# krg-nandu/monkey-pose

Hardware: NVIDIA B200
Metric: depth frames/sec (hGRU 8-step fwd) (higher is better)
Workload: dtype bf16

## Files before the change

monkey-pose_b200/csrc/hgru_lib.cu:

```cuda
#include "lib_common.cuh"

#include <cuda_bf16.h>
#include <cuda_fp16.h>
#include <cuda_runtime.h>

#include <atomic>
#include <cstdio>
#include <cstdlib>
#include <cstring>
#include <string>
#include <vector>

#include "crop.cuh"
#include "gate_tc.cuh"
#include "gemm_tc.cuh"
#include "post.cuh"
#include "hconv_tc.cuh"
#include "layers.cuh"
#include "simt_kernels.cuh"
#include <algorithm>

#include "attn.cuh"
#include "tc_host.cuh"

namespace {
thread_local std::string g_err;
int g_timing = 0;
}

namespace hgru_host {
int fail(int code, const std::string& msg) {
  g_err = msg;
  return code;
}
}

using namespace hgru_host;

namespace {

struct DevBuf {
  void* p = nullptr;
  size_t bytes = 0;
  int alloc(size_t b) {
    bytes = b;
    cudaError_t e = cudaMalloc(&p, b ? b : 16);
    if (e != cudaSuccess) return fail(HGRU_E_CUDA, std::string("cudaMalloc: ") + cudaGetErrorString(e));
    return 0;
  }
  void release() {
    if (p) cudaFree(p);
    p = nullptr;
  }
  template <class T> T* as() const { return static_cast<T*>(p); }
};

template <int KP, class Epi>
int launch_gate(const __nv_bfloat16* act, const hgru::TcConvArgs& a, cudaStream_t st) {
  using Cfg = hgru::GateCfg<KP>;
  const int tiles_per_frame = (a.H * a.W + 127) / 128;
  hgru::gate_tc_kernel<KP, Epi><<<a.N * tiles_per_frame, 128, Cfg::SMEM_BYTES, st>>>(act, a);
  CUDA_TRY(cudaGetLastError());
  return 0;
}
template <class Epi>
int dispatch_gate(int KP, const __nv_bfloat16* act, const hgru::TcConvArgs& a, cudaStream_t st) {
  if (KP == 64) return launch_gate<64, Epi>(act, a, st);
  if (KP == 32) return launch_gate<32, Epi>(act, a, st);
  if (KP == 16) return launch_gate<16, Epi>(act, a, st);
  return fail(HGRU_E_UNSUPPORTED, "tensor-core gate: unsupported padded channel count");
}

template <int S>
int launch_simt_conv(const float* in, const float* w, const float* bias, const float* scale,
                     const float* shift, float* out, int N, int H, int W, int Ci, int Co, int relu,
                     cudaStream_t st) {
  using Cfg = hgru::ConvSimtCfg<S>;
  auto kern = hgru::conv_simt_kernel<S>;
  SMEM_ATTR_ONCE(kern, Cfg::kSmemBytes);
  dim3 grid(((W + 15) / 16) * ((H + 15) / 16), (Co + 63) / 64, N);
  kern<<<grid, 256, Cfg::kSmemBytes, st>>>(in, w, bias, scale, shift, out, N, H, W, Ci, Co, relu);
  CUDA_TRY(cudaGetLastError());
  return 0;
}

int dispatch_simt_conv(int S, const float* in, const float* w, const float* bias, const float* scale,
                       const float* shift, float* out, int N, int H, int W, int Ci, int Co, int relu,
                       cudaStream_t st) {
  switch (S) {
    case 1: return launch_simt_conv<1>(in, w, bias, scale, shift, out, N, H, W, Ci, Co, relu, st);
    case 3: return launch_simt_conv<3>(in, w, bias, scale, shift, out, N, H, W, Ci, Co, relu, st);
    case 5: return launch_simt_conv<5>(in, w, bias, scale, shift, out, N, H, W, Ci, Co, relu, st);
    case 7: return launch_simt_conv<7>(in, w, bias, scale, shift, out, N, H, W, Ci, Co, relu, st);
    case 9: return launch_simt_conv<9>(in, w, bias, scale, shift, out, N, H, W, Ci, Co, relu, st);
    case 11: return launch_simt_conv<11>(in, w, bias, scale, shift, out, N, H, W, Ci, Co, relu, st);
    case 13: return launch_simt_conv<13>(in, w, bias, scale, shift, out, N, H, W, Ci, Co, relu, st);
    case 15: return launch_simt_conv<15>(in, w, bias, scale, shift, out, N, H, W, Ci, Co, relu, st);
    default: return fail(HGRU_E_UNSUPPORTED, "conv: filter size must be odd and <= 15");
  }
}

__global__ void pad_matrix_kernel(const float* in, float* out, int rows, int k, int KP, int rows_pad) {
  const int i = blockIdx.x * blockDim.x + threadIdx.x;
  if (i >= rows_pad * KP) return;
  const int c = i % KP, r = i / KP;
  out[i] = (r < rows && c < k) ? in[static_cast<size_t>(r) * k + c] : 0.f;
}
__global__ void pad_hwio_kernel(const float* in, float* out, int taps, int k, int KP) {
  const size_t i = blockIdx.x * static_cast<size_t>(blockDim.x) + threadIdx.x;
  if (i >= static_cast<size_t>(taps) * KP * KP) return;
  const int co = i % KP;
  const int ci = (i / KP) % KP;
  const int t = i / (static_cast<size_t>(KP) * KP);
  out[i] = (ci < k && co < k) ? in[(static_cast<size_t>(t) * k + ci) * k + co] : 0.f;
}

struct KernelTimer {
  std::vector<cudaEvent_t> ev;
  int used = 0;
  int kernels = 0;
  bool open = false;
  void begin(cudaStream_t st) {
    if (!g_timing || open) return;
    open = true;
    while (static_cast<int>(ev.size()) < used + 2) {
      cudaEvent_t e;
      cudaEventCreate(&e);
      ev.push_back(e);
    }
    cudaEventRecord(ev[used], st);
  }
  void end(cudaStream_t st, int n = 1) {
    if (!g_timing || !open) return;
    cudaEventRecord(ev[used + 1], st);
    used += 2;
    kernels += n;
    open = false;
  }
  void reset() { used = 0; kernels = 0; open = false; }
  int collect(float* total_ms) {
    float t = 0.f;
    for (int i = 0; i + 1 < used; i += 2) {
      cudaEventSynchronize(ev[i + 1]);
      float ms = 0.f;
      cudaEventElapsedTime(&ms, ev[i], ev[i + 1]);
      t += ms;
    }
    *total_ms = t;
    return used ? kernels : 0;
  }
  ~KernelTimer() {
    for (auto e : ev) cudaEventDestroy(e);
  }
// ... 629 lines not shown
    if (int r = p->h0_tmp.alloc(static_cast<size_t>(N) * HW * HW * C * sizeof(float))) return r;
  }
  if (h->op16() && !p->h0_identity) {
    if (!p->side_st) {
      CUDA_TRY(cudaStreamCreateWithFlags(&p->side_st, cudaStreamNonBlocking));
      CUDA_TRY(cudaEventCreateWithFlags(&p->ev_fork, cudaEventDisableTiming));
      CUDA_TRY(cudaEventCreateWithFlags(&p->ev_init, cudaEventDisableTiming));
    }
    CUDA_TRY(cudaEventRecord(p->ev_fork, st));
    CUDA_TRY(cudaStreamWaitEvent(p->side_st, p->ev_fork, 0));
    if ((rc = hgru_init_state_bf16(h, H2_init, p->side_st))) return rc;
    CUDA_TRY(cudaEventRecord(p->ev_init, p->side_st));
    h->state_ready = true;
  }
  const int per = (N + nchunks - 1) / nchunks;
  const size_t pix = static_cast<size_t>(HW) * HW;
  auto conv1 = [&](int n0, int nn) {
    float* o32 = tc ? nullptr : p->pool1.as<float>() + static_cast<size_t>(n0) * pix * KP;
    __nv_bfloat16* o16 = tc ? p->act_pool1.as<__nv_bfloat16>() + static_cast<size_t>(n0) * 2 * KP * pix : nullptr;
    hgru::stem_conv1_pool_bn_kernel<<<dim3(nblk(static_cast<size_t>(nn) * HW * ((HW + hgru::kStemPix - 1) / hgru::kStemPix)), KP / 8),
                                      256, 0, st>>>(
        depth + static_cast<size_t>(n0) * 4 * pix, p->w1.as<float>(), p->b1.as<float>(), p->bn_scale(0), p->bn_shift(0),
        o32, o16, nn, HW, HW, C, KP, tc ? 1 : 0);
    ++p->launches;
  };
  auto conv23_tc = [&](int n0, int nn) -> int {
    hgru::TcConvArgs a{};
    a.N = nn; a.n0 = n0; a.H = HW; a.W = HW; a.KP = KP; a.kreal = C;
    a.wpk = p->wpk2.as<__nv_bfloat16>(); a.bias = p->b2.as<float>();
    a.scale = p->bn_scale(1); a.shift = p->bn_shift(1);
    a.out = nullptr; a.out_bf16 = p->act_conv2.as<__nv_bfloat16>();
    int r = tc_stem_launch(KP, p->map_pool1, a, st);
    if (r) return r;
    a.wpk = p->wpk3.as<__nv_bfloat16>(); a.bias = p->b3.as<float>();
    a.scale = p->bn_scale(2); a.shift = p->bn_shift(2);
    a.out = h->Xp.as<float>(); a.out_bf16 = nullptr;
    p->launches += 2;
    return tc_stem_launch(KP, p->map_conv2, a, st);
  };
  for (int c = 0; c < nchunks; ++c) {
    const int n0 = c * per, nn = (n0 + per <= N ? per : N - n0);
    if (nn <= 0) break;
    if (chunk_ready) CUDA_TRY(cudaStreamWaitEvent(st, chunk_ready[c], 0));
    conv1(n0, nn);
    if (tc && (rc = conv23_tc(n0, nn))) return rc;
  }
  if (!tc) {
    if ((rc = dispatch_simt_conv(3, p->pool1.as<float>(), p->w2.as<float>(), p->b2.as<float>(), p->bn_scale(1),
                                 p->bn_shift(1), p->conv2.as<float>(), N, HW, HW, KP, KP, 1, st)))
      return rc;
    if ((rc = dispatch_simt_conv(3, p->conv2.as<float>(), p->w3.as<float>(), p->b3.as<float>(), p->bn_scale(2),
                                 p->bn_shift(2), h->Xp.as<float>(), N, HW, HW, KP, KP, 1, st)))
      return rc;
    p->launches += 2;
  }
  if (p->fc1_tc) {
    h->fc_a = p->fc1_a.as<__nv_bfloat16>(); h->fc_scale = p->bn_scale(3); h->fc_shift = p->bn_shift(3);
    h->fc_kpad = p->fc_kpad;
  }
  if (p->h0_identity) {
    state_to_nhwc(h, h->Xp.as<float>(), p->h0_tmp.as<float>(), st);
    H2_init = p->h0_tmp.as<float>();
    ++p->launches;
  } else if (h->op16()) {
    CUDA_TRY(cudaStreamWaitEvent(st, p->ev_init, 0));
  }
  if ((rc = hgru_run_padded(h, h->Xp.as<float>(), H2_init, nullptr, nullptr, st))) return rc;
  p->launches += h->launches;
  const int K = HW * HW * C;
  int nsplit = p->nsplit;
  if (p->fc1_tc) {
    hgru::GemmArgs g{N, p->F, K, p->fc_kpad, p->fc_kbps, p->part.as<float>(), 0, 0, 0, 0, 0, 0};
    dim3 grid((p->F + hgru::kGemmBN - 1) / hgru::kGemmBN, (N + hgru::kGemmBM - 1) / hgru::kGemmBM, p->fc_splits);
    hgru::gemm_tc_splitk_kernel<hgru::kGemmBN><<<grid, 256, hgru::kGemmSmemBytes, st>>>(p->map_fc_a, p->map_fc_a, p->map_fc_b, g);
    nsplit = p->fc_splits;
    ++p->launches;
  } else {
    const int kslice = round_up((K + p->nsplit - 1) / p->nsplit, 16);
    dim3 g1((p->F + 63) / 64, (N + 63) / 64, p->nsplit);
    hgru::fc1_splitk_kernel<<<g1, 256, 0, st>>>(h->H2.as<float>(), p->fc1_w.as<float>(), p->bn_scale(3),
                                                p->bn_shift(3), p->part.as<float>(), N, K, p->F, C, KP, kslice);
    ++p->launches;
  }
  hgru::fc_tail_kernel<<<N, 256, sizeof(float) * (p->F + hgru::kFcTailScratch), st>>>(
      p->part.as<float>(), nsplit, p->fc1_b.as<float>(), p->bn_scale(4), p->bn_shift(4),
      p->fc2_w.as<float>(), p->fc2_b.as<float>(), p->fc1.as<float>(), out, N, p->F, p->O);
  ++p->launches;
  CUDA_TRY(cudaGetLastError());
  return 0;
}

#include "attn_plan.inl"

extern "C" {

const char* hgru_last_error(void) { return g_err.c_str(); }
int hgru_version(void) { return 100; }
int hgru_enable_kernel_timing(int on) {
  g_timing = on ? 1 : 0;
  return 0;
}

int hgru_plan_create(int N, int H, int W, int k, int S, int T, int mode, hgru_plan_t* out) {
  if (!out) return fail(HGRU_E_INVALID, "hgru_plan_create: out is null");
  *out = nullptr;
  hgru_plan_s* p = new hgru_plan_s();
  int rc = hgru_plan_init(p, N, H, W, k, S, T, mode);
  if (!rc && cudaDeviceSynchronize() != cudaSuccess)
    rc = fail(HGRU_E_CUDA, "hgru_plan_create: device synchronisation failed");
  if (rc) {
    hgru_plan_free(p);
    delete p;
    return rc;
  }
  *out = p;
  return 0;
}

int hgru_plan_destroy(hgru_plan_t plan) {
  if (!plan) return 0;
  hgru_plan_free(plan);
  delete plan;
  return 0;
}

int hgru_set_params(hgru_plan_t plan, const float* p_r, const float* i_r, const float* i_b,
                    const float* o_r, const float* o_b, const float* beta, const float* nu,
                    const float* gamma, const float* kappa, const float* omega, const float* rho,
                    const float* lateral_bias, void* stream) {
  if (!plan) return fail(HGRU_E_INVALID, "hgru_set_params: null plan");
  return hgru_set_params_impl(plan, p_r, i_r, i_b, o_r, o_b, beta, nu, gamma, kappa, omega, rho,
                              lateral_bias, static_cast<cudaStream_t>(stream));
}

int hgru_forward(hgru_plan_t p, const float* X, const float* H2_init, float* H2_out, float* H1_trace,
                 float* H2_trace, void* stream) {
  if (!p) return fail(HGRU_E_INVALID, "hgru_forward: null plan");
  if (!X || !H2_out) return fail(HGRU_E_INVALID, "hgru_forward: null tensor pointer");
  cudaStream_t st = static_cast<cudaStream_t>(stream);
  state_from_nhwc(p, X, p->Xp.as<float>(), st);
  int rc = hgru_run_padded(p, p->Xp.as<float>(), H2_init, H1_trace, H2_trace, st);
  if (rc) return rc;
  state_to_nhwc(p, p->H2.as<float>(), H2_out, st);
  p->launches += 3;
  CUDA_TRY(cudaGetLastError());
  return 0;
}

size_t hgru_plan_workspace_bytes(hgru_plan_t plan) { return plan ? plan->workspace() : 0; }
int hgru_plan_launch_count(hgru_plan_t plan) { return plan ? plan->launches : 0; }

int pose_plan_create(int N, int HW, int C, int S, int T, int F, int O, int mode, pose_plan_t* out) {
  if (!out) return fail(HGRU_E_INVALID, "pose_plan_create: out is null");
  *out = nullptr;
  if (N < 1 || HW < 1 || C < 1 || F < 1 || O < 1) return fail(HGRU_E_INVALID, "pose_plan_create: non-positive shape");
  pose_plan_s* p = new pose_plan_s();
  p->N = N; p->HW = HW; p->C = C; p->S = S; p->T = T; p->F = F; p->O = O; p->mode = mode;
  int rc = hgru_plan_init(&p->hg, N, HW, HW, C, S, T, mode);
  const int KP = p->hg.KP;
  p->KP = KP;
  p->bnw = F > KP ? F : KP;
  const size_t act = static_cast<size_t>(N) * HW * HW * KP * sizeof(float);
  const size_t K = static_cast<size_t>(HW) * HW * C;
  auto A = [&](DevBuf& b, size_t bytes) { if (!rc) rc = b.alloc(bytes); };
  A(p->depth, static_cast<size_t>(N) * 4 * HW * HW * sizeof(float));
  if (mode == HGRU_MODE_FP32) { A(p->pool1, act); A(p->conv2, act); }
  A(p->w1, sizeof(float) * 9 * C); A(p->b1, sizeof(float) * KP);
  A(p->b2, sizeof(float) * KP); A(p->b3, sizeof(float) * KP);
  p->fc1_tc = (mode != HGRU_MODE_FP32);
// ... 526 lines not shown
```

monkey-pose_b200/csrc/simt_kernels.cuh:

```cuda
#pragma once
#include <cuda_bf16.h>
#include <cuda_fp16.h>
#include <cuda_runtime.h>

#include <cstdint>

#include "op_format.cuh"

namespace hgru {

__device__ __forceinline__ float sigmoidf_(float x) { return 1.f / (1.f + __expf(-x)); }
__device__ __forceinline__ float tanhf_(float x) { return tanhf(x); }

template <int S>
struct ConvSimtCfg {
  static constexpr int PH = 16 + S - 1;
  static constexpr int PWraw = 16 + S - 1;
  static constexpr int PW = ((8 + ((8 + S - 1 + 3) / 4) * 4) + 3) / 4 * 4;
  static constexpr int NWIN = ((8 + S - 1 + 3) / 4) * 4;
  static constexpr int kPatchFloats = 8 * PH * PW;
  static constexpr int kWFloats = S * 8 * 64;
  static constexpr int kSmemBytes = (kPatchFloats + kWFloats) * 4;
};

template <int S>
__global__ void __launch_bounds__(256)
conv_simt_kernel(const float* __restrict__ in, const float* __restrict__ w,
                 const float* __restrict__ bias, const float* __restrict__ scale,
                 const float* __restrict__ shift, float* __restrict__ out, int N, int H, int W,
                 int Ci, int Co, int relu) {
  using Cfg = ConvSimtCfg<S>;
  extern __shared__ float smem_f[];
  float* patch = smem_f;
  float* wsm = smem_f + Cfg::kPatchFloats;
  constexpr int PAD = (S - 1) / 2;
  const int tiles_x = (W + 15) / 16;
  const int tx = blockIdx.x % tiles_x, ty = blockIdx.x / tiles_x;
  const int co0 = blockIdx.y * 64;
  const int n = blockIdx.z;
  const int tid = threadIdx.x;
  const int cg = tid & 7;
  const int pg = tid >> 3;
  const int prow = pg >> 1;
  const int pxg = (pg & 1) * 8;
  const int y_base = ty * 16 - PAD, x_base = tx * 16 - PAD;

  float acc[8][8];
#pragma unroll
  for (int j = 0; j < 8; ++j)
#pragma unroll
    for (int c = 0; c < 8; ++c) acc[j][c] = 0.f;

  for (int ci0 = 0; ci0 < Ci; ci0 += 8) {
    __syncthreads();
    for (int e = tid; e < Cfg::PH * Cfg::PWraw * 8; e += 256) {
      const int ci = e & 7;
      const int p = e >> 3;
      const int px = p % Cfg::PWraw, py = p / Cfg::PWraw;
      const int y = y_base + py, x = x_base + px;
      float v = 0.f;
      if (y >= 0 && y < H && x >= 0 && x < W && ci0 + ci < Ci)
        v = in[((static_cast<size_t>(n) * H + y) * W + x) * Ci + ci0 + ci];
      patch[(ci * Cfg::PH + py) * Cfg::PW + px] = v;
    }
    for (int dy = 0; dy < S; ++dy) {
      __syncthreads();
      for (int e = tid; e < S * 8 * 64; e += 256) {
        const int co = e & 63;
        const int ci = (e >> 6) & 7;
        const int dx = e >> 9;
        float v = 0.f;
        if (ci0 + ci < Ci && co0 + co < Co)
          v = w[((static_cast<size_t>(dy) * S + dx) * Ci + ci0 + ci) * Co + co0 + co];
        wsm[e] = v;
      }
      __syncthreads();
#pragma unroll 1
      for (int ci = 0; ci < 8; ++ci) {
        float win[Cfg::NWIN];
        const float4* src =
            reinterpret_cast<const float4*>(patch + (ci * Cfg::PH + prow + dy) * Cfg::PW + pxg);
#pragma unroll
        for (int j = 0; j < Cfg::NWIN / 4; ++j) {
          const float4 v = src[j];
          win[4 * j] = v.x; win[4 * j + 1] = v.y; win[4 * j + 2] = v.z; win[4 * j + 3] = v.w;
        }
#pragma unroll
        for (int dx = 0; dx < S; ++dx) {
          const float4* wp = reinterpret_cast<const float4*>(wsm + (dx * 8 + ci) * 64 + cg * 8);
          const float4 w0 = wp[0], w1 = wp[1];
// ... 472 lines not shown
        const int c = cg * 8 + j;
        g.v[j] = (c < k) ? sigmoidf_(acc[i][j] + bg[c]) : 0.f;
        const float a = g.v[j] * xin[pp * (KP + 1) + c];
        hi.v[j] = __bfloat162float(__float2bfloat16(a));
        lo.v[j] = a - hi.v[j];
      }
      if (out_g) {
        float* o = out_g + ((n * (KP >> 2) + 2 * cg) * HW + pin) * 4;
        *reinterpret_cast<float4*>(o) = make_float4(g.v[0], g.v[1], g.v[2], g.v[3]);
        *reinterpret_cast<float4*>(o + static_cast<size_t>(HW) * 4) = make_float4(g.v[4], g.v[5], g.v[6], g.v[7]);
      }
      if (out_act && lo_off) {
        st8_stacked(out_act, static_cast<int>(n), cg, CG, pin, HW, W, act_pad, hi);
        st8_stacked(out_act + lo_off, static_cast<int>(n), cg, CG, pin, HW, W, act_pad, lo);
      } else if (out_act) {
        st8_bf16(chunk_ptr(out_act, static_cast<int>(n), cg, pin, HW, 2 * CG), hi);
        st8_bf16(chunk_ptr(out_act, static_cast<int>(n), CG + cg, pin, HW, 2 * CG), lo);
      }
    }
  }
}

__global__ void __launch_bounds__(256)
fc1_splitk_kernel(const float* __restrict__ A, const float* __restrict__ Wt,
                  const float* __restrict__ sc, const float* __restrict__ sh,
                  float* __restrict__ part, int M, int K, int Nout, int kch, int KP, int kslice) {
  __shared__ float As[16][64 + 4];
  __shared__ float Bs[16][64 + 4];
  const int tid = threadIdx.x;
  const int j0 = blockIdx.x * 64, m0 = blockIdx.y * 64, z = blockIdx.z;
  const int kb = z * kslice, ke = min(K, kb + kslice);
  const int tm = (tid >> 4) * 4, tj = (tid & 15) * 4;
  float acc[4][4] = {};
  for (int k0 = kb; k0 < ke; k0 += 16) {
    {
      const int r = tid >> 2, kk = (tid & 3) * 4;
      const int m = m0 + r;
#pragma unroll
      for (int q = 0; q < 4; ++q) {
        const int kidx = k0 + kk + q;
        float v = 0.f;
        if (m < M && kidx < ke) {
          const int pix = kidx / kch, c = kidx - pix * kch;
          v = A[(static_cast<size_t>(m) * (K / kch) + pix) * KP + c] * sc[c] + sh[c];
        }
        As[kk + q][r] = v;
      }
    }
    {
      const int kk = tid >> 4, jj = (tid & 15) * 4;
      const int kidx = k0 + kk;
#pragma unroll
      for (int q = 0; q < 4; ++q) {
        const int j = j0 + jj + q;
        Bs[kk][jj + q] = (kidx < ke && j < Nout) ? Wt[static_cast<size_t>(kidx) * Nout + j] : 0.f;
      }
    }
    __syncthreads();
#pragma unroll
    for (int kk = 0; kk < 16; ++kk) {
      float a[4], b[4];
#pragma unroll
      for (int q = 0; q < 4; ++q) { a[q] = As[kk][tm + q]; b[q] = Bs[kk][tj + q]; }
#pragma unroll
      for (int q = 0; q < 4; ++q)
#pragma unroll
        for (int r = 0; r < 4; ++r) acc[q][r] = fmaf(a[q], b[r], acc[q][r]);
    }
    __syncthreads();
  }
#pragma unroll
  for (int q = 0; q < 4; ++q) {
    const int m = m0 + tm + q;
    if (m >= M) continue;
#pragma unroll
    for (int r = 0; r < 4; ++r) {
      const int j = j0 + tj + r;
      if (j < Nout) part[(static_cast<size_t>(z) * M + m) * Nout + j] = acc[q][r];
    }
  }
}

constexpr int kFcTailScratch = 256;
__global__ void __launch_bounds__(256)
fc_tail_kernel(const float* __restrict__ part, int nsplit, const float* __restrict__ b1,
               const float* __restrict__ sc, const float* __restrict__ sh,
               const float* __restrict__ W2, const float* __restrict__ b2, float* __restrict__ fc1_out,
               float* __restrict__ out, int M, int Hid, int Nout) {
  extern __shared__ float r[];
  float* scratch = r + Hid;
  const int m = blockIdx.x;
  const size_t zs = static_cast<size_t>(M) * Hid;
  if ((Hid & 3) == 0) {
    for (int j = 4 * threadIdx.x; j < Hid; j += 4 * blockDim.x) {
      const float* pj = part + static_cast<size_t>(m) * Hid + j;
      float4 a = make_float4(0.f, 0.f, 0.f, 0.f);
      int z = 0;
      for (; z + 6 <= nsplit; z += 6) {
        float4 v[6];
#pragma unroll
        for (int q = 0; q < 6; ++q) v[q] = __ldg(reinterpret_cast<const float4*>(pj + (z + q) * zs));
#pragma unroll
        for (int q = 0; q < 6; ++q) { a.x += v[q].x; a.y += v[q].y; a.z += v[q].z; a.w += v[q].w; }
      }
      for (; z < nsplit; ++z) {
        const float4 v = __ldg(reinterpret_cast<const float4*>(pj + z * zs));
        a.x += v.x; a.y += v.y; a.z += v.z; a.w += v.w;
      }
      const float av[4] = {a.x, a.y, a.z, a.w};
#pragma unroll
      for (int q = 0; q < 4; ++q) {
        const float t = av[q] + b1[j + q];
        if (fc1_out) fc1_out[static_cast<size_t>(m) * Hid + j + q] = t;
        r[j + q] = fmaxf(t, 0.f) * sc[j + q] + sh[j + q];
      }
    }
  } else {
    for (int j = threadIdx.x; j < Hid; j += blockDim.x) {
      const float* pj = part + static_cast<size_t>(m) * Hid + j;
      float a = 0.f;
      for (int z = 0; z < nsplit; ++z) a += pj[z * zs];
      a += b1[j];
      if (fc1_out) fc1_out[static_cast<size_t>(m) * Hid + j] = a;
      r[j] = fmaxf(a, 0.f) * sc[j] + sh[j];
    }
  }
  __syncthreads();
  for (int o0 = 0; o0 < Nout; o0 += kFcTailScratch) {
    const int no = min(Nout - o0, kFcTailScratch);
    const int G = kFcTailScratch / no;
    const int g = threadIdx.x / no, o = threadIdx.x - g * no;
    if (g < G) {
      const float* wcol = W2 + o0 + o;
      float acc[4] = {0.f, 0.f, 0.f, 0.f};
      int j = g;
      for (; j + 15 * G < Hid; j += 16 * G) {
        float w[16];
#pragma unroll
        for (int q = 0; q < 16; ++q) w[q] = __ldg(wcol + static_cast<size_t>(j + q * G) * Nout);
#pragma unroll
        for (int q = 0; q < 16; ++q) acc[q & 3] = fmaf(r[j + q * G], w[q], acc[q & 3]);
      }
      for (; j < Hid; j += G) acc[0] = fmaf(r[j], __ldg(wcol + static_cast<size_t>(j) * Nout), acc[0]);
      scratch[g * no + o] = (acc[0] + acc[1]) + (acc[2] + acc[3]);
    }
    __syncthreads();
    if (threadIdx.x < no) {
      float a = 0.f;
      for (int gg = 0; gg < G; ++gg) a += scratch[gg * no + threadIdx.x];
      out[static_cast<size_t>(m) * Nout + o0 + threadIdx.x] = a + b2[o0 + threadIdx.x];
    }
    __syncthreads();
  }
}

__global__ void bn_fold_kernel(const float* gamma, const float* beta, const float* mean,
                               const float* var, float eps, float* scale, float* shift, int c) {
  const int i = blockIdx.x * blockDim.x + threadIdx.x;
  if (i >= c) return;
  const float s = gamma[i] / sqrtf(var[i] + eps);
  scale[i] = s;
  shift[i] = beta[i] - mean[i] * s;
}

template <class F = OpBf16>
__global__ void pack_weights_kernel(const float* __restrict__ w, typename F::T* __restrict__ wpk,
                                    int taps, int k, int ksteps, int co_pad, int ci_wrap = 0) {
  const size_t i = blockIdx.x * static_cast<size_t>(blockDim.x) + threadIdx.x;
  const size_t total = static_cast<size_t>(ksteps) * taps * 2 * co_pad * 8;
  if (i >= total) return;
  const int j = i & 7;
  size_t r = i >> 3;
  const int co = r % co_pad; r /= co_pad;
  const int ch = r & 1; r >>= 1;
  const int tap = r % taps;
  const int q = r / taps;
  int ci = q * 16 + ch * 8 + j;
  if (ci_wrap > 0 && ci >= ci_wrap) ci -= ci_wrap;
  float v = 0.f;
  if (ci < k && co < k) v = w[(static_cast<size_t>(tap) * k + ci) * k + co];
  wpk[i] = F::cvt(v);
}

template <class F = OpBf16>
__global__ void pack_weights_pairtap_kernel(const float* __restrict__ w, typename F::T* __restrict__ wpk, int k,
                                            int ksteps) {
  const size_t i = blockIdx.x * static_cast<size_t>(blockDim.x) + threadIdx.x;
  const size_t total = static_cast<size_t>(ksteps) * 15 * 8 * 2 * 128 * 8;
  if (i >= total) return;
  const int j = i & 7;
  size_t r = i >> 3;
  const int row = r % 128; r /= 128;
  const int ch = r & 1; r >>= 1;
  const int b = r % 8; r /= 8;
  const int dy = r % 15;
  const int q = static_cast<int>(r / 15);
  int dx = -1;
  if (b == 0) { if (row < 64) dx = 7; }
  else dx = (row < 64) ? (b - 1 + 8) : (b - 1);
  const int co = row & 63;
  const int ci = q * 16 + ch * 8 + j;
  float v = 0.f;
  if (dx >= 0 && ci < k && co < k) v = w[((static_cast<size_t>(dy) * 15 + dx) * k + ci) * k + co];
  wpk[i] = F::cvt(v);
}

__global__ void pack_weights_split3_kernel(const float* __restrict__ w, __nv_bfloat16* __restrict__ wpk,
                                           int taps, int k, int ksteps, int co_pad) {
  const size_t i = blockIdx.x * static_cast<size_t>(blockDim.x) + threadIdx.x;
  const size_t group = static_cast<size_t>(3) * taps * 2 * co_pad * 8;
  if (i >= group * ksteps) return;
  const int q = static_cast<int>(i / group);
  size_t r = i - q * group;
  const size_t wide_elems = static_cast<size_t>(taps) * 2 * (2 * co_pad) * 8;
  int tap, ch, n, j, lo;
  if (r < wide_elems) {
    j = r & 7; r >>= 3;
    n = r % (2 * co_pad); r /= (2 * co_pad);
    ch = r & 1; tap = static_cast<int>(r >> 1);
    lo = n >= co_pad;
    if (lo) n -= co_pad;
  } else {
    r -= wide_elems;
    j = r & 7; r >>= 3;
    n = r % co_pad; r /= co_pad;
    ch = r & 1; tap = static_cast<int>(r >> 1);
    lo = 0;
  }
  const int ci = q * 16 + ch * 8 + j;
  float v = 0.f;
  if (ci < k && n < k) v = w[(static_cast<size_t>(tap) * k + ci) * k + n];
  const __nv_bfloat16 hi = __float2bfloat16(v);
  wpk[i] = lo ? __float2bfloat16(v - __bfloat162float(hi)) : hi;
// ... 4 lines not shown
```

monkey-pose_b200/csrc/sm100_ptx.cuh:

```cuda
#pragma once
#include <cstdint>
#include <cuda.h>

namespace sm100 {

__device__ __forceinline__ uint32_t smem_u32(const void* p) {
  return static_cast<uint32_t>(__cvta_generic_to_shared(p));
}

__device__ __forceinline__ bool elect_one() {
  uint32_t pred;
  asm volatile(
      "{\n\t.reg .pred p;\n\t"
      "elect.sync _|p, 0xffffffff;\n\t"
      "selp.u32 %0, 1, 0, p;\n\t}"
      : "=r"(pred));
  return pred != 0;
}

__device__ __forceinline__ void mbar_init(uint32_t bar, uint32_t count) {
  asm volatile("mbarrier.init.shared::cta.b64 [%0], %1;" ::"r"(bar), "r"(count) : "memory");
}
__device__ __forceinline__ void fence_barrier_init() {
  asm volatile("fence.mbarrier_init.release.cluster;" ::: "memory");
}
__device__ __forceinline__ void fence_proxy_async() {
  asm volatile("fence.proxy.async.shared::cta;" ::: "memory");
}
__device__ __forceinline__ void grid_launch_dependents() { asm volatile("griddepcontrol.launch_dependents;" ::: "memory"); }
__device__ __forceinline__ int ld_acquire_gpu(const int* p) {
  int v;
  asm volatile("ld.acquire.gpu.global.s32 %0, [%1];" : "=r"(v) : "l"(p) : "memory");
  return v;
}
__device__ __forceinline__ void fence_proxy_async_global() { asm volatile("fence.proxy.async.global;" ::: "memory"); }
__device__ __forceinline__ void mbar_arrive(uint32_t bar) {
  asm volatile("mbarrier.arrive.shared::cta.b64 _, [%0];" ::"r"(bar) : "memory");
}
__device__ __forceinline__ void mbar_arrive_expect_tx(uint32_t bar, uint32_t bytes) {
  asm volatile("mbarrier.arrive.expect_tx.shared::cta.b64 _, [%0], %1;" ::"r"(bar), "r"(bytes)
               : "memory");
}
__device__ __forceinline__ bool mbar_try_wait(uint32_t bar, uint32_t parity) {
  uint32_t ok;
  asm volatile(
      "{\n\t.reg .pred p;\n\t"
      "mbarrier.try_wait.parity.shared::cta.b64 p, [%1], %2;\n\t"
      "selp.u32 %0, 1, 0, p;\n\t}"
      : "=r"(ok)
      : "r"(bar), "r"(parity)
      : "memory");
  return ok != 0;
}
__device__ __forceinline__ bool mbar_test(uint32_t bar, uint32_t parity) {
  uint32_t ok;
  asm volatile(
      "{\n\t.reg .pred p;\n\t"
      "mbarrier.test_wait.parity.shared::cta.b64 p, [%1], %2;\n\t"
      "selp.u32 %0, 1, 0, p;\n\t}"
      : "=r"(ok)
      : "r"(bar), "r"(parity)
      : "memory");
  return ok != 0;
}
__device__ __forceinline__ void mbar_wait(uint32_t bar, uint32_t parity) {
  while (!mbar_try_wait(bar, parity)) {
  }
}
__device__ __forceinline__ void mbar_wait_warp(uint32_t bar, uint32_t parity) {
  while (!__all_sync(0xffffffffu, mbar_try_wait(bar, parity))) {
  }
}

__device__ __forceinline__ void tma_prefetch_desc(const CUtensorMap* m) {
  asm volatile("prefetch.tensormap [%0];" ::"l"(reinterpret_cast<uint64_t>(m)) : "memory");
}
__device__ __forceinline__ void tma_load_4d(uint32_t dst, const CUtensorMap* m, uint32_t bar,
                                            int c0, int c1, int c2, int c3) {
  asm volatile(
      "cp.async.bulk.tensor.4d.shared::cluster.global.mbarrier::complete_tx::bytes"
      " [%0], [%1, {%3, %4, %5, %6}], [%2];"
      ::"r"(dst), "l"(reinterpret_cast<uint64_t>(m)), "r"(bar), "r"(c0), "r"(c1), "r"(c2), "r"(c3)
      : "memory");
}
__device__ __forceinline__ void tma_load_2d(uint32_t dst, const CUtensorMap* m, uint32_t bar,
                                            int c0, int c1) {
  asm volatile(
      "cp.async.bulk.tensor.2d.shared::cluster.global.mbarrier::complete_tx::bytes"
      " [%0], [%1, {%3, %4}], [%2];"
      ::"r"(dst), "l"(reinterpret_cast<uint64_t>(m)), "r"(bar), "r"(c0), "r"(c1)
      : "memory");
}
__device__ __forceinline__ void bulk_load(uint32_t dst, const void* src, uint32_t bytes,
                                          uint32_t bar) {
  asm volatile(
      "cp.async.bulk.shared::cluster.global.mbarrier::complete_tx::bytes [%0], [%1], %2, [%3];"
      ::"r"(dst), "l"(reinterpret_cast<uint64_t>(src)), "r"(bytes), "r"(bar)
      : "memory");
}

template <uint32_t kCols>
__device__ __forceinline__ void tmem_alloc(uint32_t slot_smem) {
  asm volatile("tcgen05.alloc.cta_group::1.sync.aligned.shared::cta.b32 [%0], %1;"
               ::"r"(slot_smem), "n"(kCols) : "memory");
  asm volatile("tcgen05.relinquish_alloc_permit.cta_group::1.sync.aligned;" ::: "memory");
}
template <uint32_t kCols>
__device__ __forceinline__ void tmem_dealloc(uint32_t taddr) {
  asm volatile("tcgen05.dealloc.cta_group::1.sync.aligned.b32 %0, %1;" ::"r"(taddr), "n"(kCols)
               : "memory");
}
__device__ __forceinline__ void tc_fence_before() {
// ... 121 lines not shown
```

Measured before the change: 51950.

## Batch multiple frames per fc tail block and chain it with programmatic launch

The readout tail kernel now handles up to four frames per block with 512 threads. Two thread halves each cover interleaved frames, so every loaded FC2 weight is reused across several frames instead of being re-read per frame. The kernel is launched with programmatic stream serialization after the tensor-core split-K GEMM and waits on griddepcontrol, which lets its launch overlap the GEMM tail. Unroll depths for the split-sum and weight loops are also increased. The cost is more shared memory and registers per block and fewer blocks in the grid. A profiling script is also added.

```diff
diff --git a/monkey-pose_b200/csrc/devtools/step_breakdown.py b/monkey-pose_b200/csrc/devtools/step_breakdown.py
--- /dev/null
+++ b/monkey-pose_b200/csrc/devtools/step_breakdown.py
@@ -0,0 +1,148 @@
+import argparse
+import json
+import os
+import subprocess
+import sys
+import tempfile
+
+sys.path.insert(0, os.path.join(os.path.dirname(os.path.abspath(__file__)), "..", "..", ".."))
+import torch
+from torch.profiler import ProfilerActivity, profile
+
+import monkey_pose_b200 as mp
+from monkey_pose_b200 import initialization as init
+
+
+def gpu_info():
+    q = "name,power.limit,clocks.max.sm"
+    try:
+        row = subprocess.run(["nvidia-smi", "-i", str(torch.cuda.current_device()), "--query-gpu=" + q,
+                              "--format=csv,noheader"], capture_output=True, text=True, timeout=30).stdout.strip()
+        name, power, clk = [x.strip() for x in row.split(",")]
+        return {"gpu": name, "power_limit": power, "sm_clock_max": clk}
+    except Exception as e:
+        return {"gpu": torch.cuda.get_device_name(), "power_limit": "unknown (%r)" % e, "sm_clock_max": None}
+
+
+def phase_of(name, seen_hgru):
+    if "init_state" in name:
+        return "init"
+    if "stem_conv1" in name:
+        return "conv1"
+    if "hconv_stack_kernel" in name:
+        return "hgru"
+    if "hconv_tc_kernel" in name:
+        return "hgru" if seen_hgru else "conv23"
+    if "gemm_tc_splitk" in name:
+        return "fc1"
+    if "fc_tail" in name:
+        return "tail"
+    return "other"
+
+
+def median(xs):
+    xs = sorted(xs)
+    return xs[len(xs) // 2] if xs else None
+
+
+def main():
+    ap = argparse.ArgumentParser()
+    ap.add_argument("--batch", type=int, default=256)
+    ap.add_argument("--channels", type=int, default=25)
+    ap.add_argument("--timesteps", type=int, default=8)
+    ap.add_argument("--mode", default="bf16")
+    ap.add_argument("--steps", type=int, default=20)
+    ap.add_argument("--warmup", type=int, default=5)
+    ap.add_argument("--out", help="also write the result as JSON to this file")
+    a = ap.parse_args()
+    assert torch.cuda.is_available(), "step_breakdown.py measures on a CUDA device"
+
+    P = init.pose_params(channels=a.channels, S=15, T=a.timesteps, hw=64, fc_hidden=1024, out=69, seed=3)
+    depth = torch.as_tensor(init.synthetic_depth(a.batch, seed=1234)).cuda()
+    m = mp.model()
+    m.channels, m.timesteps, m.compute_mode = a.channels, a.timesteps, a.mode
+    m.hidden_state = torch.as_tensor(init.hidden_init((a.batch, 64, 64, a.channels), seed=5)).cuda()
+    m.load_params(P)
+    for _ in range(a.warmup):
+        m.build(depth, 69)
+    torch.cuda.synchronize()
+
+    e0, e1 = torch.cuda.Event(enable_timing=True), torch.cuda.Event(enable_timing=True)
+    e0.record()
+    for _ in range(a.steps):
+        m.build(depth, 69)
+    e1.record()
+    torch.cuda.synchronize()
+    step_ms = e0.elapsed_time(e1) / a.steps
+
+    with profile(activities=[ProfilerActivity.CUDA]) as prof:
+        for _ in range(a.steps):
+            torch.cuda._sleep(100)
+            m.build(depth, 69)
+        torch.cuda._sleep(100)
+        torch.cuda.synchronize()
+    with tempfile.TemporaryDirectory() as d:
+        trace = os.path.join(d, "trace.json")
+        prof.export_chrome_trace(trace)
+        with open(trace) as f:
+            events = json.load(f)["traceEvents"]
+    kern = sorted((e for e in events if e.get("cat") == "kernel"), key=lambda e: e["ts"])
+    steps, cur = [], None
+    for e in kern:
+        if "spin_kernel" in e["name"]:
+            if cur:
+                steps.append(cur)
+            cur = []
+        elif cur is not None:
+            cur.append(e)
+    per_step = []
+    for ks in steps:
+        seen_hgru, rows = False, []
+        for e in ks:
+            ph = phase_of(e["name"], seen_hgru)
+            seen_hgru |= ph == "hgru"
+            rows.append((ph, float(e["ts"]), float(e["ts"]) + float(e["dur"])))
+        if not any(r[0] == "hgru" for r in rows):
+            continue
+        t_first = min(r[1] for r in rows)
+        busy = {}
+        for ph, s, t in rows:
+            b = busy.setdefault(ph, [0.0, 0])
+            b[0] += t - s
+            b[1] += 1
+        hg = [r for r in rows if r[0] == "hgru"]
+        h0, h1 = min(r[1] for r in hg), max(r[2] for r in hg)
+        fc_end = max((r[2] for r in rows if r[0] == "fc1"), default=h1)
+        end = max(r[2] for r in rows)
+        per_step.append({"busy_us": {k: v[0] for k, v in busy.items()},
+                         "launches": {k: v[1] for k, v in busy.items()},
+                         "path_us": {"pre_hgru": h0 - t_first, "hgru": h1 - h0, "fc1": fc_end - h1,
+                                     "tail": end - fc_end, "step": end - t_first}})
+    phases = sorted({k for s in per_step for k in s["busy_us"]})
+    res = dict(gpu_info())
+    res.update({
+        "workload": "pose forward, batch %d, %d channels, T=%d, %s, device-resident crops" % (
+            a.batch, a.channels, a.timesteps, a.mode),
+        "step_ms_events": step_ms,
+        "profiled_steps": len(per_step),
+        "busy_us_median": {p: median([s["busy_us"].get(p, 0.0) for s in per_step]) for p in phases},
+        "launches_per_step": {p: per_step[0]["launches"].get(p, 0) for p in phases} if per_step else {},
+        "critical_path_us_median": {k: median([s["path_us"][k] for s in per_step])
+                                    for k in ("pre_hgru", "hgru", "fc1", "tail", "step")},
+        "note": "busy: summed kernel durations of the phase (side-stream kernels overlap others); critical path: "
+                "stretches of the device timeline of one step under torch.profiler; step_ms_events: CUDA events "
+                "over %d back-to-back forwards without the profiler" % a.steps})
+    print("%s, power limit %s" % (res["gpu"], res["power_limit"]))
+    print("step (events, no profiler): %.3f ms" % step_ms)
+    print("phase     launches   busy us (median of %d steps)" % len(per_step))
+    for p in phases:
+        print("  %-7s %8d %12.1f" % (p, res["launches_per_step"].get(p, 0), res["busy_us_median"][p]))
+    print("critical path us: " + "  ".join("%s %.1f" % kv for kv in res["critical_path_us_median"].items()))
+    if a.out:
+        with open(a.out, "w") as f:
+            json.dump(res, f, indent=1)
+    print(json.dumps(res))
+
+
+if __name__ == "__main__":
+    main()
diff --git a/monkey-pose_b200/csrc/hgru_lib.cu b/monkey-pose_b200/csrc/hgru_lib.cu
--- a/monkey-pose_b200/csrc/hgru_lib.cu
+++ b/monkey-pose_b200/csrc/hgru_lib.cu
@@ -69,6 +69,31 @@
   if (KP == 32) return launch_gate<32, Epi>(act, a, st);
   if (KP == 16) return launch_gate<16, Epi>(act, a, st);
   return fail(HGRU_E_UNSUPPORTED, "tensor-core gate: unsupported padded channel count");
+}
+
+constexpr size_t kMaxSmemPerBlock = 227 * 1024;
+template <int MT>
+int launch_fc_tail_mt(const float* part, int nsplit, const float* b1, const float* sc, const float* sh, const float* W2,
+                      const float* b2, float* fc1_out, float* out, int N, int Hid, int Nout, bool chain, cudaStream_t st) {
+  auto kern = hgru::fc_tail_kernel<MT>;
+  SMEM_ATTR_ONCE(kern, kMaxSmemPerBlock);
+  cudaLaunchConfig_t cfg{};
+  cfg.gridDim = dim3((N + MT - 1) / MT); cfg.blockDim = dim3(hgru::kFcTailThreads);
+  cfg.dynamicSmemBytes = hgru::fc_tail_smem_bytes<MT>(Hid); cfg.stream = st;
+  cudaLaunchAttribute at[1];
+  at[0].id = cudaLaunchAttributeProgrammaticStreamSerialization;
+  at[0].val.programmaticStreamSerializationAllowed = 1;
+  cfg.attrs = at; cfg.numAttrs = chain ? 1 : 0;
+  CUDA_TRY(cudaLaunchKernelEx(&cfg, kern, part, nsplit, b1, sc, sh, W2, b2, fc1_out, out, N, Hid, Nout));
+  return 0;
+}
+int launch_fc_tail(const float* part, int nsplit, const float* b1, const float* sc, const float* sh, const float* W2,
+                   const float* b2, float* fc1_out, float* out, int N, int Hid, int Nout, bool chain, cudaStream_t st) {
+  if (hgru::fc_tail_smem_bytes<4>(Hid) <= kMaxSmemPerBlock)
+    return launch_fc_tail_mt<4>(part, nsplit, b1, sc, sh, W2, b2, fc1_out, out, N, Hid, Nout, chain, st);
+  if (hgru::fc_tail_smem_bytes<1>(Hid) <= kMaxSmemPerBlock)
+    return launch_fc_tail_mt<1>(part, nsplit, b1, sc, sh, W2, b2, fc1_out, out, N, Hid, Nout, chain, st);
+  return fail(HGRU_E_UNSUPPORTED, "readout tail: hidden width too large for shared memory");
 }
 
 template <int S>
@@ -864,9 +889,10 @@
                                                 p->bn_shift(3), p->part.as<float>(), N, K, p->F, C, KP, kslice);
     ++p->launches;
   }
-  hgru::fc_tail_kernel<<<N, 256, sizeof(float) * (p->F + hgru::kFcTailScratch), st>>>(
-      p->part.as<float>(), nsplit, p->fc1_b.as<float>(), p->bn_scale(4), p->bn_shift(4),
-      p->fc2_w.as<float>(), p->fc2_b.as<float>(), p->fc1.as<float>(), out, N, p->F, p->O);
+  if ((rc = launch_fc_tail(p->part.as<float>(), nsplit, p->fc1_b.as<float>(), p->bn_scale(4), p->bn_shift(4),
+                           p->fc2_w.as<float>(), p->fc2_b.as<float>(), p->fc1.as<float>(), out, N, p->F, p->O,
+                           p->fc1_tc, st)))
+    return rc;
   ++p->launches;
   CUDA_TRY(cudaGetLastError());
   return 0;
diff --git a/monkey-pose_b200/csrc/simt_kernels.cuh b/monkey-pose_b200/csrc/simt_kernels.cuh
--- a/monkey-pose_b200/csrc/simt_kernels.cuh
+++ b/monkey-pose_b200/csrc/simt_kernels.cuh
@@ -6,6 +6,7 @@
 #include <cstdint>
 
 #include "op_format.cuh"
+#include "sm100_ptx.cuh"
 
 namespace hgru {
 
@@ -644,26 +645,39 @@
 }
 
 constexpr int kFcTailScratch = 256;
-__global__ void __launch_bounds__(256)
+constexpr int kFcTailThreads = 2 * kFcTailScratch;
+template <int MT>
+constexpr size_t fc_tail_smem_bytes(int Hid) { return sizeof(float) * MT * (static_cast<size_t>(Hid) + kFcTailScratch); }
+template <int MT>
+__global__ void __launch_bounds__(kFcTailThreads)
 fc_tail_kernel(const float* __restrict__ part, int nsplit, const float* __restrict__ b1,
                const float* __restrict__ sc, const float* __restrict__ sh,
                const float* __restrict__ W2, const float* __restrict__ b2, float* __restrict__ fc1_out,
                float* __restrict__ out, int M, int Hid, int Nout) {
+  constexpr int FH = (MT + 1) / 2;
   extern __shared__ float r[];
-  float* scratch = r + Hid;
-  const int m = blockIdx.x;
+  float* scratch = r + MT * Hid;
+  const int m0 = blockIdx.x * MT;
+  const int nf = min(MT, M - m0);
+  sm100::grid_dependency_wait();
   const size_t zs = static_cast<size_t>(M) * Hid;
   if ((Hid & 3) == 0) {
-    for (int j = 4 * threadIdx.x; j < Hid; j += 4 * blockDim.x) {
+    const int h4 = Hid / 4;
+    for (int i = threadIdx.x; i < MT * h4; i += blockDim.x) {
+      const int f = i / h4, j = 4 * (i - f * h4), m = m0 + f;
+      if (f >= nf) {
+        *reinterpret_cast<float4*>(r + f * Hid + j) = make_float4(0.f, 0.f, 0.f, 0.f);
+        continue;
+      }
       const float* pj = part + static_cast<size_t>(m) * Hid + j;
       float4 a = make_float4(0.f, 0.f, 0.f, 0.f);
       int z = 0;
-      for (; z + 6 <= nsplit; z += 6) {
-        float4 v[6];
-#pragma unroll
-        for (int q = 0; q < 6; ++q) v[q] = __ldg(reinterpret_cast<const float4*>(pj + (z + q) * zs));
-#pragma unroll
-        for (int q = 0; q < 6; ++q) { a.x += v[q].x; a.y += v[q].y; a.z += v[q].z; a.w += v[q].w; }
+      for (; z + 9 <= nsplit; z += 9) {
+        float4 v[9];
+#pragma unroll
+        for (int q = 0; q < 9; ++q) v[q] = __ldg(reinterpret_cast<const float4*>(pj + (z + q) * zs));
+#pragma unroll
+        for (int q = 0; q < 9; ++q) { a.x += v[q].x; a.y += v[q].y; a.z += v[q].z; a.w += v[q].w; }
       }
       for (; z < nsplit; ++z) {
         const float4 v = __ldg(reinterpret_cast<const float4*>(pj + z * zs));
@@ -674,43 +688,73 @@
       for (int q = 0; q < 4; ++q) {
         const float t = av[q] + b1[j + q];
         if (fc1_out) fc1_out[static_cast<size_t>(m) * Hid + j + q] = t;
-        r[j + q] = fmaxf(t, 0.f) * sc[j + q] + sh[j + q];
+        r[f * Hid + j + q] = fmaxf(t, 0.f) * sc[j + q] + sh[j + q];
       }
     }
   } else {
-    for (int j = threadIdx.x; j < Hid; j += blockDim.x) {
+    for (int i = threadIdx.x; i < MT * Hid; i += blockDim.x) {
+      const int f = i / Hid, j = i - f * Hid, m = m0 + f;
+      if (f >= nf) {
+        r[i] = 0.f;
+        continue;
+      }
       const float* pj = part + static_cast<size_t>(m) * Hid + j;
       float a = 0.f;
       for (int z = 0; z < nsplit; ++z) a += pj[z * zs];
       a += b1[j];
       if (fc1_out) fc1_out[static_cast<size_t>(m) * Hid + j] = a;
-      r[j] = fmaxf(a, 0.f) * sc[j] + sh[j];
+      r[i] = fmaxf(a, 0.f) * sc[j] + sh[j];
     }
   }
   __syncthreads();
+  const int h = threadIdx.x / kFcTailScratch, th = threadIdx.x - h * kFcTailScratch;
   for (int o0 = 0; o0 < Nout; o0 += kFcTailScratch) {
     const int no = min(Nout - o0, kFcTailScratch);
     const int G = kFcTailScratch / no;
-    const int g = threadIdx.x / no, o = threadIdx.x - g * no;
-    if (g < G) {
+    const int g = th / no, o = th - g * no;
+    if (g < G && h < MT) {
       const float* wcol = W2 + o0 + o;
-      float acc[4] = {0.f, 0.f, 0.f, 0.f};
+      const float* rh = r + h * Hid;
+      float acc[FH][4];
+#pragma unroll
+      for (int k = 0; k < FH; ++k)
+#pragma unroll
+        for (int q = 0; q < 4; ++q) acc[k][q] = 0.f;
       int j = g;
+      for (; j + 47 * G < Hid; j += 48 * G) {
+        float w[48];
+#pragma unroll
+        for (int q = 0; q < 48; ++q) w[q] = __ldg(wcol + static_cast<size_t>(j + q * G) * Nout);
+#pragma unroll
+        for (int k = 0; k < FH; ++k)
+#pragma unroll
+          for (int q = 0; q < 48; ++q) acc[k][q & 3] = fmaf(rh[2 * k * Hid + j + q * G], w[q], acc[k][q & 3]);
+      }
       for (; j + 15 * G < Hid; j += 16 * G) {
         float w[16];
 #pragma unroll
         for (int q = 0; q < 16; ++q) w[q] = __ldg(wcol + static_cast<size_t>(j + q * G) * Nout);
 #pragma unroll
-        for (int q = 0; q < 16; ++q) acc[q & 3] = fmaf(r[j + q * G], w[q], acc[q & 3]);
-      }
-      for (; j < Hid; j += G) acc[0] = fmaf(r[j], __ldg(wcol + static_cast<size_t>(j) * Nout), acc[0]);
-      scratch[g * no + o] = (acc[0] + acc[1]) + (acc[2] + acc[3]);
+        for (int k = 0; k < FH; ++k)
+#pragma unroll
+          for (int q = 0; q < 16; ++q) acc[k][q & 3] = fmaf(rh[2 * k * Hid + j + q * G], w[q], acc[k][q & 3]);
+      }
+      for (; j < Hid; j += G) {
+        const float w = __ldg(wcol + static_cast<size_t>(j) * Nout);
+#pragma unroll
+        for (int k = 0; k < FH; ++k) acc[k][0] = fmaf(rh[2 * k * Hid + j], w, acc[k][0]);
+      }
+#pragma unroll
+      for (int k = 0; k < FH; ++k)
+        if (h + 2 * k < MT)
+          scratch[(h + 2 * k) * kFcTailScratch + g * no + o] = (acc[k][0] + acc[k][1]) + (acc[k][2] + acc[k][3]);
     }
     __syncthreads();
-    if (threadIdx.x < no) {
+    for (int i = threadIdx.x; i < nf * no; i += blockDim.x) {
+      const int f = i / no, oo = i - f * no;
       float a = 0.f;
-      for (int gg = 0; gg < G; ++gg) a += scratch[gg * no + threadIdx.x];
-      out[static_cast<size_t>(m) * Nout + o0 + threadIdx.x] = a + b2[o0 + threadIdx.x];
+      for (int gg = 0; gg < G; ++gg) a += scratch[f * kFcTailScratch + gg * no + oo];
+      out[static_cast<size_t>(m0 + f) * Nout + o0 + oo] = a + b2[o0 + oo];
     }
     __syncthreads();
   }
diff --git a/monkey-pose_b200/csrc/sm100_ptx.cuh b/monkey-pose_b200/csrc/sm100_ptx.cuh
--- a/monkey-pose_b200/csrc/sm100_ptx.cuh
+++ b/monkey-pose_b200/csrc/sm100_ptx.cuh
@@ -28,6 +28,7 @@
   asm volatile("fence.proxy.async.shared::cta;" ::: "memory");
 }
 __device__ __forceinline__ void grid_launch_dependents() { asm volatile("griddepcontrol.launch_dependents;" ::: "memory"); }
+__device__ __forceinline__ void grid_dependency_wait() { asm volatile("griddepcontrol.wait;" ::: "memory"); }
 __device__ __forceinline__ int ld_acquire_gpu(const int* p) {
   int v;
   asm volatile("ld.acquire.gpu.global.s32 %0, [%1];" : "=r"(v) : "l"(p) : "memory");
```

After: 51610 (median of 6 runs). Within noise of the previous version (-0.7%).
